# LeCAR-Lab/dial-mpc

Hardware: NVIDIA H100
Metric: sample-steps/s (Nsample*Hsample/wall-s) per MPC reverse_once, Go2 (higher is better)
Workload: dtype f32

## Files before the change

### dial_mpc_b200/csrc/dial_kernels.cu

```cuda
#include <cuda_runtime.h>
#include <stdio.h>
#include <stdlib.h>
#include <float.h>
#include <cmath>
#include <memory>
#include <string>
#include <vector>
#include <new>
#include "dial_host.h"
#define DIAL_STR2(x) #x
#define DIAL_STR(x) DIAL_STR2(x)

static thread_local std::string g_err;
static int fail(const std::string& s) { g_err = s; return -1; }
#define CUDA_OK(x) do { cudaError_t e_ = (x); if (e_ != cudaSuccess) return fail(std::string(#x) + ": " + cudaGetErrorString(e_)); } while (0)

#ifdef DIAL_ONLY_VARIANT
#define DIAL_HAS_VARIANT(v) ((v) == DIAL_ONLY_VARIANT)
#define DIAL_VARIANT DIAL_ONLY_VARIANT
#include "dial_rollout_variant.cu"
#else
#define DIAL_HAS_VARIANT(v) 1
#endif
#define DIAL_DECL_LAUNCH(v) cudaError_t dial_launch_rollout_v##v(const DevModel*, const DevPlan*, const RolloutArgs&, int, int, size_t, cudaStream_t);
// ... 346 lines not shown
  }
  if (tid == 0) {
    *counter = 0u;
    uint32_t n0, n1;
    split_rng(r0, r1, n0, n1);
    rng[0] = n0; rng[1] = n1;
    if (X.mbox) *X.seq = *X.seq + 1u;
  }
}

__global__ void mpc_split_kernel(uint32_t* __restrict__ rng, uint32_t* __restrict__ key) {
  if (threadIdx.x == 0) {
    const uint32_t k0 = rng[0], k1 = rng[1];
    uint32_t a0 = 0, b0 = 2, a1 = 1, b1 = 3;
    threefry2x32(k0, k1, a0, b0);
    threefry2x32(k0, k1, a1, b1);
    rng[0] = a0; rng[1] = a1; key[0] = b0; key[1] = b1;
  }
}

__global__ void mpc_shift_kernel(const float* __restrict__ Msh, const float* __restrict__ Yin,
                                 float* __restrict__ Yout, int n1, int nu) {
  const int i = threadIdx.x;
  Yin += (size_t)blockIdx.x * n1 * nu; Yout += (size_t)blockIdx.x * n1 * nu;
  if (i < n1 * nu) {
    const int k = i / nu, a = i - k * nu;
    float s = 0.f;
    for (int j = 0; j < n1; ++j) s += Msh[k * n1 + j] * Yin[j * nu + a];
    Yout[i] = s;
  }
}

#define TB_CHUNKS 32
struct TrajArgs {
  const float* traj[3];
  float* out[3];
  int ncol[3], coloff[3];
  int coltot, nrows, H;
  int inst_rows;
  const float* weights;
  int w_offset, mean_row, mean_weight_index, include_mean;
  float* partial;
};

template <bool BATCH>
__global__ void __launch_bounds__(256, 8) trajbar_partial_kernel(const TrajArgs T, const int32_t* __restrict__ iter_lim, int iter) {
  const int chunk = blockIdx.y, arr = BATCH ? blockIdx.z % 3 : blockIdx.z, inst = BATCH ? blockIdx.z / 3 : 0;
  const int ncol = arr == 0 ? T.ncol[0] : (arr == 1 ? T.ncol[1] : T.ncol[2]), len = T.H * ncol;
  const int coloff = arr == 0 ? T.coloff[0] : (arr == 1 ? T.coloff[1] : T.coloff[2]);
  const int j = blockIdx.x * 256 + threadIdx.x;
  if (blockIdx.x * 256 >= len || (BATCH && !schedule_runs(iter_lim, inst, iter))) return;
  const float* __restrict__ traj = (arr == 0 ? T.traj[0] : (arr == 1 ? T.traj[1] : T.traj[2])) + (size_t)inst * T.inst_rows * len;
  const float* wts = BATCH ? T.weights + (size_t)inst * (T.mean_weight_index + 1) : T.weights;
  const int per = (T.nrows + TB_CHUNKS - 1) / TB_CHUNKS;
  const int r0 = chunk * per, r1 = min(T.nrows, r0 + per);
  const int jj = j < len ? j : len - 1;
  float a = 0.f;
  for (int r = r0; r < r1; r += 8) {
    float wv[8], xv[8];
#pragma unroll
    for (int k = 0; k < 8; ++k) {
      const int rr = r + k;
      float wgt = 0.f;
      if (rr < r1) {
        if (rr == T.mean_row) wgt = T.include_mean ? wts[T.mean_weight_index] : 0.f;
        else wgt = wts[T.w_offset + rr];
      }
      wv[k] = wgt;
    }
#pragma unroll
    for (int k = 0; k < 8; ++k)
      xv[k] = (wv[k] != 0.f) ? traj[(size_t)(r + k) * len + jj] : 0.f;
#pragma unroll
    for (int k = 0; k < 8; ++k) a += wv[k] * xv[k];
  }
  if (j < len) {
    const int t = j / ncol, c = j - t * ncol;
    T.partial[(((size_t)inst * TB_CHUNKS + chunk) * T.H + t) * T.coltot + coloff + c] = a;
  }
}

template <bool BATCH>
__global__ void __launch_bounds__(128, 8) trajbar_final_kernel(const TrajArgs T, const int32_t* __restrict__ iter_lim, int iter) {
  const int t = blockIdx.x, inst = BATCH ? blockIdx.y : 0;
  if (BATCH && !schedule_runs(iter_lim, inst, iter)) return;
  const float* partial = T.partial + (size_t)inst * TB_CHUNKS * T.H * T.coltot;
  for (int col = threadIdx.x; col < T.coltot; col += blockDim.x) {
    float s = 0.f;
#pragma unroll 8
    for (int ch = 0; ch < TB_CHUNKS; ++ch) s += partial[((size_t)ch * T.H + t) * T.coltot + col];
    float* out; int ncol, off;
    if (col >= T.coloff[2]) { out = T.out[2]; ncol = T.ncol[2]; off = T.coloff[2]; }
    else if (col >= T.coloff[1]) { out = T.out[1]; ncol = T.ncol[1]; off = T.coloff[1]; }
    else { out = T.out[0]; ncol = T.ncol[0]; off = T.coloff[0]; }
    if (out) out[((size_t)inst * T.H + t) * ncol + (col - off)] = s;
  }
}

__global__ void __launch_bounds__(256) ensemble_reduce_kernel(const float* __restrict__ r, const EnsRisk* __restrict__ risk,
                                                              const EnsAdapt* __restrict__ adapt, const float* __restrict__ belief,
                                                              int K, int n1, float* __restrict__ rews,
                                                              const int32_t* __restrict__ iter_lim, int iter) {
  const int i = blockIdx.x * blockDim.x + threadIdx.x, b = blockIdx.y;
  if (i >= n1 || !schedule_runs(iter_lim, b, iter)) return;
  const EnsRisk R = risk[b];
  const float* rb = r + (size_t)b * K * n1 + i;
  rews[(size_t)b * n1 + i] = adapt[b].on ? ens_risk_reduce_weighted(rb, (size_t)n1, K, R, belief + (size_t)b * K, adapt[b].prune)
                                         : ens_risk_reduce(rb, (size_t)n1, K, R);
}

__global__ void __launch_bounds__(128) ens_gather_kernel(const float* __restrict__ Y, int K, int n1, int nu,
// ... 122 lines not shown
    ev.clear();
    cudaFree(d); cudaFreeHost(h);
    d = nullptr; h = nullptr;
  }
};

struct LaunchKey {
  bool models = false, members = false, sched = false, lims = false, adapt = false, delay = false, obs = false;
  bool predicts = false;
  int npred = 0;
  bool planning() const { return obs || npred > 0; }
  bool operator!=(const LaunchKey& o) const {
    return models != o.models || members != o.members || sched != o.sched || lims != o.lims || adapt != o.adapt ||
           delay != o.delay || obs != o.obs || predicts != o.predicts || npred != o.npred;
  }
};

struct dial_plan {
  DevModel hM;
  DevPlan hP;
  DevModel* dM = nullptr;
  DevPlan* dP = nullptr;
  int variant = 0;
  int shape = 0;
  int n_inst = 1;
  int n_ens = 0;
  int num_sms = 132;
  size_t smem_bytes = 0;
  float *traj_q[2] = {nullptr, nullptr}, *traj_qd[2] = {nullptr, nullptr}, *traj_x[2] = {nullptr, nullptr};
  int cur = 0;
  float* weights = nullptr;
  float* weights2 = nullptr;
  cudaStream_t side = nullptr;
  cudaEvent_t ev_main[2] = {nullptr, nullptr}, ev_side[2] = {nullptr, nullptr};
  float* partial = nullptr;
  float* tb_partial = nullptr;
  unsigned int* counter = nullptr;
  unsigned int* row_counter = nullptr;
  float* zeros = nullptr;
  int ybar_grid = 0;
  int upd_grid = 0;
  int64_t launches = 0;
  float* dbg = nullptr;
  dial_mpc_buffers mpc{};
  bool mpc_bound = false;
  float* mpc_Msh = nullptr;
  float* mpc_Y1 = nullptr;
  uint32_t* mpc_key = nullptr;
  struct MpcGraph { int n_diffuse, env_step, seen; cudaGraphExec_t exec; int64_t launches; };
  std::vector<MpcGraph> mpc_graphs;
  LaunchKey key, ran;
  Staged<DevModel> models;
  Staged<DevModel> members;
  float* ens_rews = nullptr;
  Staged<EnsRisk> risk;
  Staged<EnsAdapt> adapt;
  Staged<double> belief_L;
  Staged<float> belief_w;
  float* dEll = nullptr;
  float* pred_us = nullptr;
  float* pred_qd = nullptr;
  Staged<InstSchedule> sched;
  Staged<int32_t> lims;
  struct PlanningState {
    float *qpos = nullptr, *qvel = nullptr, *warm = nullptr;
    int32_t* cnt = nullptr;
// ... 57 lines not shown
static void fill_xch(const dial_plan* p, RolloutArgs& A) {
  if (!p->xch.on) return;
  A.xch_world = p->xch.world; A.xch_rank = p->xch.rank;
  for (int r = 0; r < p->xch.world; ++r) { A.xch_mbox[r] = p->xch.mbox(r); A.xch_flags[r] = p->xch.flags(r); }
  A.xch_seq = p->xch.seq(); A.xch_done = p->xch.done();
}
static XchWait xch_wait_args(const dial_plan* p, float* rews_copy) {
  XchWait X; memset(&X, 0, sizeof(X));
  if (p->xch.on) {
    X.mbox = p->xch.mbox(p->xch.rank); X.flags = p->xch.flags(p->xch.rank); X.seq = p->xch.seq(); X.err = p->xch.err();
    X.rews_copy = rews_copy; X.world = p->xch.world;
  }
  return X;
}

extern "C" int dial_abi_version(void) { return DIAL_ABI_VERSION; }
extern "C" const char* dial_last_error(void) { return g_err.c_str(); }
extern "C" size_t dial_sizeof(int which) {
  return which == 0 ? sizeof(dial_model_desc) : which == 1 ? sizeof(dial_plan_desc) : which == 2 ? sizeof(dial_state)
       : which == 3 ? sizeof(dial_mpc_buffers) : which == 4 ? sizeof(dial_task) : 0;
}

static cudaError_t launch_rollout(dial_plan* p, const RolloutArgs& A, int wpc, cudaStream_t st) {
  const size_t smem = sizeof(DevModel) + sizeof(DevPlan) + (size_t)wpc * p->hM.warp_floats * sizeof(float);
  int grid = (A.nrows + wpc - 1) / wpc;
  if (A.models && model_rows(A) > 0) grid = (A.nrows / model_rows(A)) * ((model_rows(A) + wpc - 1) / wpc);
  if (A.row_counter) {
    const int resident = p->num_sms * (wpc > 8 ? 1 : 16 / wpc);
    grid = grid < resident ? grid : resident;
    cudaError_t e = cudaMemsetAsync(A.row_counter, 0, sizeof(unsigned int), st);
    if (e != cudaSuccess) return e;
  }
  p->launches++;
#ifndef DIAL_ONLY_VARIANT
  if (p->shape > 0) return kShapes[p->shape - 1].launch(p->dM, p->dP, A, grid, wpc, smem, st);
#endif
  switch (p->variant) {
#if DIAL_HAS_VARIANT(1)
    case 1: return dial_launch_rollout_v1(p->dM, p->dP, A, grid, wpc, smem, st);
#endif
#if DIAL_HAS_VARIANT(2)
    case 2: return dial_launch_rollout_v2(p->dM, p->dP, A, grid, wpc, smem, st);
#endif
#if DIAL_HAS_VARIANT(3)
    case 3: return dial_launch_rollout_v3(p->dM, p->dP, A, grid, wpc, smem, st);
#endif
#if DIAL_HAS_VARIANT(4)
    case 4: return dial_launch_rollout_v4(p->dM, p->dP, A, grid, wpc, smem, st);
#endif
#if DIAL_HAS_VARIANT(0)
    case 0: return dial_launch_rollout_v0(p->dM, p->dP, A, grid, wpc, smem, st);
#endif
    default: return cudaErrorInvalidDeviceFunction;
  }
}

static int default_wpc(const dial_plan* p, int nrows) {
  const int per_sm = (nrows + p->num_sms - 1) / p->num_sms;
  const size_t fixed = sizeof(DevModel) + sizeof(DevPlan), slab = (size_t)p->hM.warp_floats * sizeof(float);
  int maxw = DIAL_MAXTHREADS / 32;
  while (maxw > 1 && fixed + maxw * slab > 227 * 1024) --maxw;
  if (per_sm <= maxw) return per_sm;
  const int waves = (per_sm + maxw - 1) / maxw;
  return (per_sm + waves - 1) / waves;
}

// ... 77 lines not shown
      if (kShapes[s].matches(p->hM, p->hP.c)) { p->shape = s + 1; break; }
#endif
  auto bad = [&](cudaError_t e, const char* what) {
    g_err = std::string(what) + ": " + cudaGetErrorString(e);
    dial_plan_destroy(p);
    return (dial_plan*)nullptr;
  };
  cudaError_t e = cudaSuccess;
  if (p->own(e, p->dM, sizeof(DevModel)) != cudaSuccess) return bad(e, "cudaMalloc(model)");
  if (p->own(e, p->dP, sizeof(DevPlan)) != cudaSuccess) return bad(e, "cudaMalloc(plan)");
  if ((e = cudaMemcpy(p->dM, &p->hM, sizeof(DevModel), cudaMemcpyHostToDevice)) != cudaSuccess) return bad(e, "cudaMemcpy(model)");
  if ((e = cudaMemcpy(p->dP, &p->hP, sizeof(DevPlan), cudaMemcpyHostToDevice)) != cudaSuccess) return bad(e, "cudaMemcpy(plan)");
  const size_t B = (size_t)p->n_inst, H = (size_t)c.Hsample + 1;
  const size_t rows = B * (p->n_ens > 1 ? (size_t)p->n_ens : 1) * ((size_t)c.Nsample + 1);
  const dial_model_desc& m = *model;
  for (int b = 0; b < 2; ++b) {
    if (p->own(e, p->traj_q[b], rows * H * m.nq * sizeof(float)) != cudaSuccess) return bad(e, "cudaMalloc(traj_q)");
    if (p->own(e, p->traj_qd[b], rows * H * m.nv * sizeof(float)) != cudaSuccess) return bad(e, "cudaMalloc(traj_qd)");
    if (p->own(e, p->traj_x[b], rows * H * 3 * (m.nbody - 1) * sizeof(float)) != cudaSuccess) return bad(e, "cudaMalloc(traj_x)");
  }
  if (p->n_ens > 1) {
    if (p->own(e, p->ens_rews, rows * sizeof(float)) != cudaSuccess) return bad(e, "cudaMalloc(ens_rews)");
    const size_t K = p->n_ens;
    const double L0 = log(1.0 / p->n_ens);
    if ((e = p->risk.allocate(B, 1, ens_risk_derive(p->n_ens, DIAL_ENS_MEAN, 1.f))) != cudaSuccess) return bad(e, "allocate(risk)");
    if ((e = p->adapt.allocate(B, 1, EnsAdapt{})) != cudaSuccess) return bad(e, "allocate(adapt)");
    if ((e = p->belief_L.allocate(B, K, L0)) != cudaSuccess) return bad(e, "allocate(belief)");
    if ((e = p->belief_w.allocate(B, K, (float)exp(L0))) != cudaSuccess) return bad(e, "allocate(belief)");
    if (p->own(e, p->dEll, B * K * sizeof(float)) != cudaSuccess) return bad(e, "cudaMalloc(belief)");
    if ((e = cudaMemset(p->dEll, 0, B * K * sizeof(float))) != cudaSuccess) return bad(e, "cudaMemset(belief)");
  }
  if (p->own(e, p->weights, B * ((size_t)c.Ntotal + 1) * sizeof(float)) != cudaSuccess) return bad(e, "cudaMalloc(weights)");
  if (p->own(e, p->weights2, B * ((size_t)c.Ntotal + 1) * sizeof(float)) != cudaSuccess) return bad(e, "cudaMalloc(weights2)");
  if ((e = cudaStreamCreateWithFlags(&p->side, cudaStreamNonBlocking)) != cudaSuccess) return bad(e, "cudaStreamCreate(side)");
  for (int i = 0; i < 2; ++i) {
    if ((e = cudaEventCreateWithFlags(&p->ev_main[i], cudaEventDisableTiming)) != cudaSuccess) return bad(e, "cudaEventCreate");
    if ((e = cudaEventCreateWithFlags(&p->ev_side[i], cudaEventDisableTiming)) != cudaSuccess) return bad(e, "cudaEventCreate");
  }
  const int ne = (c.Hnode + 1) * m.nu, slots = YBAR_THREADS / ne;
  int g = (c.Ntotal + 1 + slots - 1) / slots;
  p->ybar_grid = g < 1 ? 1 : (g > 2 * p->num_sms ? 2 * p->num_sms : g);
  {
    int gu = (c.Ntotal + 1 + slots * 8 - 1) / (slots * 8);
    p->upd_grid = gu < 1 ? 1 : (gu > p->ybar_grid ? p->ybar_grid : gu);
  }
  if (p->own(e, p->partial, B * p->ybar_grid * (ne + 1) * sizeof(float)) != cudaSuccess) return bad(e, "cudaMalloc(partial)");
  if (p->own(e, p->tb_partial, B * TB_CHUNKS * H * (m.nq + m.nv + 3 * (m.nbody - 1)) * sizeof(float)) != cudaSuccess) return bad(e, "cudaMalloc(tb_partial)");
  if (p->own(e, p->counter, B * sizeof(unsigned int)) != cudaSuccess) return bad(e, "cudaMalloc(counter)");
  if ((e = cudaMemset(p->counter, 0, B * sizeof(unsigned int))) != cudaSuccess) return bad(e, "cudaMemset(counter)");
  if (p->own(e, p->row_counter, sizeof(unsigned int)) != cudaSuccess) return bad(e, "cudaMalloc(row_counter)");
  if (getenv("DIAL_DEBUG_COUNTERS")) {
    if (p->own(e, p->dbg, 8 * sizeof(float)) != cudaSuccess) return bad(e, "cudaMalloc(dbg)");
    cudaMemset(p->dbg, 0, 8 * sizeof(float));
  }
  if (p->own(e, p->zeros, DIAL_MAXV * sizeof(float)) != cudaSuccess) return bad(e, "cudaMalloc(zeros)");
  if ((e = cudaMemset(p->zeros, 0, DIAL_MAXV * sizeof(float))) != cudaSuccess) return bad(e, "cudaMemset(zeros)");
  return p;
}

extern "C" void dial_plan_destroy(dial_plan* p) {
  if (!p) return;
  drop_graphs(p);
  for (int r = 0; r < DIAL_MAXRANK; ++r) {
    if (!p->xch.base[r]) continue;
    if (r == p->xch.rank) cudaFree(p->xch.base[r]); else cudaIpcCloseMemHandle(p->xch.base[r]);
  }
  cudaFree(p->xch.bars_partial);
// ... 511 lines not shown
  ybar_kernel<<<p->ybar_grid, YBAR_THREADS, 0, st>>>(w, eps, key ? key[0] : 0u, key ? key[1] : 0u, Ybar, noise_scale,
                                                     c.Ntotal, c.Hnode + 1, p->hM.m.nu, p->partial, p->counter, Ybar_out, nullptr);
  p->launches++;
  CUDA_OK(cudaGetLastError());
  if (weights && weights != p->weights)
    CUDA_OK(cudaMemcpyAsync(p->weights, weights, ((size_t)c.Ntotal + 1) * sizeof(float), cudaMemcpyDeviceToDevice, st));
  return 0;
}

static int launch_update(dial_plan* p, const float* rews, float* weights, const XchWait& X, uint32_t* rng,
                         const float* Ybar, const float* noise, float* Ybar_out, cudaStream_t st,
                         const InstSchedule* sched = nullptr, const int32_t* iter_lim = nullptr, int iter = 0,
                         const float* weights_prev = nullptr) {
  const dial_plan_desc& c = p->hP.c;
  update_kernel<<<dim3(p->upd_grid, p->n_inst), YBAR_THREADS, 0, st>>>(rews, c.Ntotal + 1, c.temp_sample, weights, X, rng, Ybar,
                                                                     noise, c.Ntotal, c.Hnode + 1, p->hM.m.nu, p->partial,
                                                                     p->counter, Ybar_out, sched, iter_lim, iter,
                                                                     weights_prev ? weights_prev : weights);
  p->launches++;
  CUDA_OK(cudaGetLastError());
  return 0;
}

extern "C" int dial_reverse_update_fused(dial_plan* p, const float* rews, uint32_t* rng, const float* Ybar,
                                         const float* noise_scale, float* Ybar_out, float* weights, void* stream) {
  if (!p || !rews || !rng || !Ybar || !noise_scale || !Ybar_out || !weights) return fail("dial_reverse_update_fused: null argument");
  const dial_plan_desc& c = p->hP.c;
  if (c.Ntotal != c.Nsample) return fail("dial_reverse_update_fused: sharded plans (Ntotal != Nsample) are not supported");
  if (c.Ntotal + 1 > (1 << 17)) return fail("dial_reverse_update_fused: needs Ntotal + 1 <= 131072 (the fused update)");
  XchWait X; memset(&X, 0, sizeof(X));
  return launch_update(p, rews, weights, X, rng, Ybar, noise_scale, Ybar_out, (cudaStream_t)stream);
}

static int enqueue_trajbar(dial_plan* p, const float* weights, int rank, float* qbar, float* qdbar, float* xbar,
                           cudaStream_t st, const int32_t* iter_lim = nullptr, int iter = 0) {
  const dial_plan_desc& c = p->hP.c;
  const dial_model_desc& m = p->hM.m;
  const float* w = weights ? weights : p->weights;
  const int H = c.Hsample + 1, rows = c.Nsample + 1;
  TrajArgs T;
  T.traj[0] = p->traj_q[p->cur]; T.traj[1] = p->traj_qd[p->cur]; T.traj[2] = p->traj_x[p->cur];
  T.out[0] = qbar; T.out[1] = qdbar; T.out[2] = xbar;
  const bool xsum = p->xch.on && qbar && qdbar && xbar;
  if (xsum) {
    T.out[0] = p->xch.bars_partial; T.out[1] = T.out[0] + (size_t)H * m.nq; T.out[2] = T.out[1] + (size_t)H * m.nv;
  }
  T.ncol[0] = m.nq; T.ncol[1] = m.nv; T.ncol[2] = 3 * (m.nbody - 1);
  T.coloff[0] = 0; T.coloff[1] = m.nq; T.coloff[2] = m.nq + m.nv;
  T.coltot = m.nq + m.nv + 3 * (m.nbody - 1);
  T.nrows = rows; T.inst_rows = (p->n_ens > 1 ? p->n_ens : 1) * rows; T.H = H; T.weights = w; T.w_offset = c.shard_offset; T.mean_row = c.Nsample;
  T.mean_weight_index = c.Ntotal; T.include_mean = rank == 0 ? 1 : 0; T.partial = p->tb_partial;
  const int maxlen = H * (T.ncol[2] > T.ncol[0] ? T.ncol[2] : T.ncol[0]);
  const dim3 g1((maxlen + 255) / 256, TB_CHUNKS, 3 * p->n_inst), g2(H, p->n_inst);
  const bool batch = p->n_inst > 1 || iter_lim;
  if (batch) trajbar_partial_kernel<true><<<g1, 256, 0, st>>>(T, iter_lim, iter);
  else trajbar_partial_kernel<false><<<g1, 256, 0, st>>>(T, nullptr, 0);
  p->launches++;
  CUDA_OK(cudaGetLastError());
  if (batch) trajbar_final_kernel<true><<<g2, 128, 0, st>>>(T, iter_lim, iter);
  else trajbar_final_kernel<false><<<g2, 128, 0, st>>>(T, nullptr, 0);
  p->launches++;
  CUDA_OK(cudaGetLastError());
  if (xsum) {
    BarsXch Bx; memset(&Bx, 0, sizeof(Bx));
    for (int r = 0; r < p->xch.world; ++r) { Bx.mbox[r] = p->xch.bars(r); Bx.flags[r] = p->xch.bflags(r); }
    Bx.seq = p->xch.bseq(); Bx.err = p->xch.err(); Bx.world = p->xch.world; Bx.rank = p->xch.rank; Bx.nbar = p->xch.nbar;
    Bx.partial = p->xch.bars_partial; Bx.out[0] = qbar; Bx.out[1] = qdbar; Bx.out[2] = xbar;
    Bx.n0 = H * m.nq; Bx.n1 = H * m.nv;
    bars_allreduce_kernel<<<1, 1024, 0, st>>>(Bx);
    p->launches++;
    CUDA_OK(cudaGetLastError());
  }
  return 0;
}

extern "C" int dial_reverse_trajbar(dial_plan* p, const float* weights, int rank, float* qbar, float* qdbar,
                                    float* xbar, void* stream) {
  if (!p) return fail("dial_reverse_trajbar: null plan");
  if (p->n_inst > 1) return fail("dial_reverse_trajbar: batched plans run through dial_mpc_step");
  return enqueue_trajbar(p, weights, rank, qbar, qdbar, xbar, (cudaStream_t)stream);
}

extern "C" int dial_exchange_create(dial_plan* p, int rank, int world, unsigned char handle_out[DIAL_IPC_HANDLE_BYTES]) {
  if (!p || !handle_out) return fail("dial_exchange_create: null argument");
  if (world < 2 || world > DIAL_MAXRANK || rank < 0 || rank >= world) return fail("dial_exchange_create: need 2 <= world <= DIAL_MAXRANK");
  static_assert(sizeof(cudaIpcMemHandle_t) <= DIAL_IPC_HANDLE_BYTES, "IPC handle does not fit");
  const dial_plan_desc& c = p->hP.c;
  const dial_model_desc& m = p->hM.m;
  if (c.Ntotal != c.Nsample * world || c.shard_offset != rank * c.Nsample) return fail("dial_exchange_create: plan shard does not match rank/world");
// ... 41 lines not shown
  if (!p || !out) return fail("dial_exchange_status: null argument");
  if (!p->xch.on) { for (int i = 0; i < 6; ++i) out[i] = 0; return 0; }
  CUDA_OK(cudaMemcpy(out, p->xch.base[p->xch.rank] + p->xch.o_local, 6 * sizeof(uint32_t), cudaMemcpyDeviceToHost));
  return 0;
}

extern "C" int dial_reverse_trajectories(dial_plan* p, float* q, float* qd, float* xpos, void* stream) {
  if (!p) return fail("dial_reverse_trajectories: null plan");
  if (p->n_inst > 1) return fail("dial_reverse_trajectories: batched plans run through dial_mpc_step");
  const dial_plan_desc& c = p->hP.c;
  const dial_model_desc& m = p->hM.m;
  const size_t n = ((size_t)c.Nsample + 1) * (c.Hsample + 1) * sizeof(float);
  cudaStream_t st = (cudaStream_t)stream;
  if (q) CUDA_OK(cudaMemcpyAsync(q, p->traj_q[p->cur], n * m.nq, cudaMemcpyDeviceToDevice, st));
  if (qd) CUDA_OK(cudaMemcpyAsync(qd, p->traj_qd[p->cur], n * m.nv, cudaMemcpyDeviceToDevice, st));
  if (xpos) CUDA_OK(cudaMemcpyAsync(xpos, p->traj_x[p->cur], n * 3 * (m.nbody - 1), cudaMemcpyDeviceToDevice, st));
  return 0;
}

extern "C" int dial_mpc_bind(dial_plan* p, const dial_mpc_buffers* b, const float* M_shift) {
  if (!p || !b || !M_shift) return fail("dial_mpc_bind: null argument");
  if (!b->qpos || !b->qvel || !b->qacc_warmstart || !b->counters || !b->rng || !b->Y || !b->ctrl || !b->reward ||
      !b->rews || !b->noise)
    return fail("dial_mpc_bind: only qbar/qdbar/xbar may be null");
  const dial_plan_desc& c = p->hP.c;
  if (c.Ntotal != c.Nsample && !p->xch.on)
    return fail("dial_mpc_bind: a sharded plan needs a connected exchange (dial_exchange_create / dial_exchange_connect) for the device-resident loop");
  if (c.Ntotal != c.Nsample && !b->rews_all) return fail("dial_mpc_bind: sharded plans need rews_all [Ntotal+1]");
  if (p->n_inst > 1 && b->rews_all) return fail("dial_mpc_bind: rews_all must be NULL on a batched plan");
  const int n1 = c.Hnode + 1, nu = p->hM.m.nu;
  drop_graphs(p);
  cudaError_t e = cudaSuccess;
  if (!p->mpc_Msh) CUDA_OK(p->own(e, p->mpc_Msh, DIAL_MAXNODE * DIAL_MAXNODE * sizeof(float)));
  if (!p->mpc_Y1) CUDA_OK(p->own(e, p->mpc_Y1, (size_t)p->n_inst * DIAL_MAXNODE * DIAL_MAXU * sizeof(float)));
  if (!p->mpc_key) CUDA_OK(p->own(e, p->mpc_key, 2 * sizeof(uint32_t)));
  CUDA_OK(cudaMemcpy(p->mpc_Msh, M_shift, (size_t)n1 * n1 * sizeof(float), cudaMemcpyHostToDevice));
  (void)nu;
  p->mpc = *b;
  p->mpc_bound = true;
  return 0;
}

static int mpc_enqueue(dial_plan* p, const LaunchKey& k, int n_diffuse, int env_step, cudaStream_t st) {
  const dial_plan_desc& c = p->hP.c;
  const dial_mpc_buffers& B = p->mpc;
  const int n1 = c.Hnode + 1, nu = p->hM.m.nu, ni = p->n_inst;
  const int K = p->n_ens > 1 ? p->n_ens : 1;
  const bool batched = ni > 1;
  const dial_plan::DelayQueue& Q = p->queue;
  const dial_plan::PlanningState& P = p->planning;
  float* Y[2] = {B.Y, p->mpc_Y1};
  int cur = 0;
  if (k.delay && (env_step == 1 || k.predicts)) {
    delay_queue_kernel<<<ni, 128, 0, st>>>(p->delay.d, Q.head, Q.ring, Y[cur], n1, nu, env_step == 1,
                                           Q.applied, Q.pending, Q.len);
    p->launches++;
    CUDA_OK(cudaGetLastError());
  }
  const float* act = k.delay ? Q.applied : Y[cur];
  const int act_n1 = k.delay ? 1 : n1;
  const bool adapt = env_step == 1 && k.adapt;
  if (adapt) {
    ens_gather_kernel<<<ni, 128, 0, st>>>(act, K, act_n1, nu, p->pred_us);
    p->launches++;
    CUDA_OK(cudaGetLastError());
    RolloutArgs A; memset(&A, 0, sizeof(A));
    A.qpos0 = B.qpos; A.qvel0 = B.qvel; A.warm0 = B.qacc_warmstart; A.counters_in = B.counters;
    A.nrows = ni * K; A.H = 1; A.mode = 0; A.us = p->pred_us;
    A.rows_per_inst = K; A.rows_per_model = 1; A.models = p->members.d;
    if (B.tasks) { A.tasks = B.tasks; A.task_rows = K; }
    A.qd = p->pred_qd;
    CUDA_OK(launch_rollout(p, A, 1, st));
  }
  if (env_step == 1) {
    RolloutArgs A; memset(&A, 0, sizeof(A));
    A.qpos0 = B.qpos; A.qvel0 = B.qvel; A.warm0 = B.qacc_warmstart;
    A.counters_in = B.counters; A.counters_out = B.counters;
    A.nrows = ni; A.H = 1; A.mode = 0; A.us = act; A.rewss = B.reward;
    if (batched) { A.rows_per_inst = 1; A.us_row = act_n1 * nu; }
    if (B.tasks) { A.tasks = B.tasks; A.task_rows = batched ? 1 : 0; }
    A.models = p->models.d;
    A.qpos_out = B.qpos; A.qvel_out = B.qvel; A.warm_out = B.qacc_warmstart; A.ctrl_out = B.ctrl;
    CUDA_OK(launch_rollout(p, A, 1, st));
  }
  if (adapt) {
    ens_belief_kernel<<<ni, 32, 0, st>>>(p->pred_qd, B.qvel, p->adapt.d, K, p->hM.m.nv, p->belief_L.d, p->belief_w.d, p->dEll);
    p->launches++;
    CUDA_OK(cudaGetLastError());
  }
  if (env_step == 1 || env_step == 2) {
    mpc_shift_kernel<<<ni, DIAL_MAXNODE * DIAL_MAXU, 0, st>>>(p->mpc_Msh, Y[cur], Y[cur ^ 1], n1, nu);
    p->launches++;
    CUDA_OK(cudaGetLastError());
    cur ^= 1;
  }
  const float *qpos0 = B.qpos, *qvel0 = B.qvel, *warm0 = B.qacc_warmstart;
  const int32_t* cnt0 = B.counters;
  if (k.obs) {
    observe_kernel<<<ni, 128, 0, st>>>(p->dM, p->obs.d, p->ob, p->delay.d, Q.pending, env_step == 1, B.qpos, B.qvel,
                                       B.qacc_warmstart, B.counters, act, act_n1 * nu, P.qpos, P.qvel, P.warm, P.cnt);
    p->launches++;
    CUDA_OK(cudaGetLastError());
  } else if (k.npred > 0) {
    const size_t nq = p->hM.m.nq, nv = p->hM.m.nv;
    CUDA_OK(cudaMemcpyAsync(P.qpos, B.qpos, ni * nq * sizeof(float), cudaMemcpyDeviceToDevice, st));
    CUDA_OK(cudaMemcpyAsync(P.qvel, B.qvel, ni * nv * sizeof(float), cudaMemcpyDeviceToDevice, st));
    CUDA_OK(cudaMemcpyAsync(P.warm, B.qacc_warmstart, ni * nv * sizeof(float), cudaMemcpyDeviceToDevice, st));
    CUDA_OK(cudaMemcpyAsync(P.cnt, B.counters, ni * 2 * sizeof(int32_t), cudaMemcpyDeviceToDevice, st));
  }
  for (int j = 0; j < k.npred; ++j) {
    RolloutArgs A; memset(&A, 0, sizeof(A));
    A.qpos0 = P.qpos; A.qvel0 = P.qvel; A.warm0 = P.warm;
    A.counters_in = P.cnt; A.counters_out = P.cnt;
    A.nrows = ni; A.H = 1; A.mode = 0; A.rows_per_inst = 1;
    A.us = (k.obs ? p->ob.seq : Q.pending) + (size_t)j * nu; A.us_row = DIAL_MAXDELAY * nu;
    if (B.tasks) { A.tasks = B.tasks; A.task_rows = batched ? 1 : 0; }
    A.models = p->n_ens > 0 ? P.models : p->models.d;
    A.iter_lim = k.obs ? p->ob.len : Q.len; A.iter = j;
    A.qpos_out = P.qpos; A.qvel_out = P.qvel; A.warm_out = P.warm;
    CUDA_OK(launch_rollout(p, A, 1, st));
  }
  if (k.planning()) { qpos0 = P.qpos; qvel0 = P.qvel; warm0 = P.warm; cnt0 = P.cnt; }
  const bool bars = B.qbar && B.qdbar && B.xbar;
  float* wts[2] = {p->weights, p->weights2};
  const size_t nw = (size_t)ni * (c.Ntotal + 1);
  for (int i = 0; i < n_diffuse; ++i) {
    const float* noise = B.noise + (size_t)i * n1;
    const bool fused = c.Ntotal + 1 <= (1 << 17) && !getenv("DIAL_NO_FUSED_UPDATE");
    if (!fused) {
      mpc_split_kernel<<<1, 32, 0, st>>>(B.rng, p->mpc_key);
      p->launches++;
      CUDA_OK(cudaGetLastError());
    }
    if (bars && i >= 2) CUDA_OK(cudaStreamWaitEvent(st, p->ev_side[i & 1], 0));
    RolloutArgs A; memset(&A, 0, sizeof(A));
    A.qpos0 = qpos0; A.qvel0 = qvel0; A.warm0 = warm0; A.counters_in = cnt0;
    A.nrows = ni * K * (c.Nsample + 1); A.H = c.Hsample + 1; A.mode = 1;
    if (batched || p->n_ens > 0) A.rows_per_inst = K * (c.Nsample + 1);
    if (B.tasks) { A.tasks = B.tasks; A.task_rows = batched ? K * (c.Nsample + 1) : 0; }
    if (p->n_ens > 0) { A.rows_per_model = c.Nsample + 1; A.models = p->members.d; }
    else A.models = p->models.d;
    A.Ybar = Y[cur]; A.noise = noise;
    A.sched = p->sched.d; A.iter_lim = p->lims.d; A.iter = i;
    if (fused) A.rng_dev = B.rng; else A.key_dev = p->mpc_key;
    p->cur ^= 1;
    A.rews = K > 1 ? p->ens_rews : B.rews; A.q = p->traj_q[p->cur]; A.qd = p->traj_qd[p->cur]; A.xpos = p->traj_x[p->cur];
    A.dbg = p->dbg;
    fill_xch(p, A);
    CUDA_OK(launch_rollout_any(p, A, st));
    if (K > 1) {
      const dim3 grid((c.Nsample + 1 + 255) / 256, ni);
      ensemble_reduce_kernel<<<grid, 256, 0, st>>>(p->ens_rews, p->risk.d, p->adapt.d, p->belief_w.d, K, c.Nsample + 1, B.rews,
                                                   p->lims.d, i);
      p->launches++;
      CUDA_OK(cudaGetLastError());
    }
    float* w = wts[i & 1];
    XchWait X = xch_wait_args(p, B.rews_all);
    if (fused) {
      int rc = launch_update(p, B.rews, w, X, B.rng, Y[cur], noise, Y[cur ^ 1], st, p->sched.d, p->lims.d, i,
                             wts[i > 0 ? (i - 1) & 1 : 0]);
      if (rc) return rc;
    } else {
      weights_kernel<<<1, 1024, 0, st>>>(B.rews, c.Ntotal + 1, c.temp_sample, w, X);
      p->launches++;
      CUDA_OK(cudaGetLastError());
      ybar_kernel<<<p->ybar_grid, YBAR_THREADS, 0, st>>>(w, nullptr, 0u, 0u, Y[cur], noise, c.Ntotal, n1, nu,
                                                         p->partial, p->counter, Y[cur ^ 1], p->mpc_key);
      p->launches++;
      CUDA_OK(cudaGetLastError());
    }
    cur ^= 1;
    if (bars) {
      CUDA_OK(cudaEventRecord(p->ev_main[i & 1], st));
      CUDA_OK(cudaStreamWaitEvent(p->side, p->ev_main[i & 1], 0));
      int rc = enqueue_trajbar(p, w, p->xch.on ? p->xch.rank : 0, B.qbar, B.qdbar, B.xbar, p->side, p->lims.d, i);
      if (rc) return rc;
      CUDA_OK(cudaEventRecord(p->ev_side[i & 1], p->side));
    }
  }
  if (cur != 0) CUDA_OK(cudaMemcpyAsync(Y[0], Y[1], (size_t)ni * n1 * nu * sizeof(float), cudaMemcpyDeviceToDevice, st));
  if (bars && n_diffuse > 0) {
    if (n_diffuse >= 2) CUDA_OK(cudaStreamWaitEvent(st, p->ev_side[(n_diffuse - 2) & 1], 0));
    CUDA_OK(cudaStreamWaitEvent(st, p->ev_side[(n_diffuse - 1) & 1], 0));
  }
  if (n_diffuse > 0 && wts[(n_diffuse - 1) & 1] != p->weights)
    CUDA_OK(cudaMemcpyAsync(p->weights, p->weights2, nw * sizeof(float), cudaMemcpyDeviceToDevice, st));
  return 0;
}

extern "C" int dial_mpc_step(dial_plan* p, int n_diffuse, int env_step, void* stream) {
  if (!p) return fail("dial_mpc_step: null plan");
  if (!p->mpc_bound) return fail("dial_mpc_step: call dial_mpc_bind first");
  if (n_diffuse < 0 || n_diffuse > 64) return fail("dial_mpc_step: n_diffuse out of range");
  if (env_step < 0 || env_step > 2) return fail("dial_mpc_step: env_step must be 0 (plan only), 1 (env step + shift) or 2 (shift only)");
  if (p->n_inst > 1 && getenv("DIAL_NO_FUSED_UPDATE")) return fail("dial_mpc_step: batched plans need the fused update (unset DIAL_NO_FUSED_UPDATE)");
  if ((p->sched.d || p->lims.d) && getenv("DIAL_NO_FUSED_UPDATE"))
    return fail("dial_mpc_step: per-instance schedules and iteration limits need the fused update (unset DIAL_NO_FUSED_UPDATE)");
  for (int b = 0; p->sched.d && b < p->n_inst; ++b) {
    const InstSchedule& S = p->sched.h[b];
    const int runs = p->lims.d && p->lims.h[b] < n_diffuse ? p->lims.h[b] : n_diffuse;
    if (S.on && runs > S.n_rows)
      return fail("dial_mpc_step: instance " + std::to_string(b) + " runs " + std::to_string(runs) +
                  " diffusion iterations, its schedule has " + std::to_string(S.n_rows) + " rows");
  }
  cudaStream_t st = (cudaStream_t)stream;
  if (p->key != p->ran) drop_graphs(p);
  p->ran = p->key;
  dial_plan::MpcGraph* g = nullptr;
  for (auto& e : p->mpc_graphs) if (e.n_diffuse == n_diffuse && e.env_step == env_step) g = &e;
  if (!g) {
    p->mpc_graphs.push_back({n_diffuse, env_step, 1, nullptr, 0});
    return mpc_enqueue(p, p->ran, n_diffuse, env_step, st);
  }
  if (!g->exec) {
    if (getenv("DIAL_NO_GRAPH")) return mpc_enqueue(p, p->ran, n_diffuse, env_step, st);
    cudaStream_t cs;
    CUDA_OK(cudaStreamCreateWithFlags(&cs, cudaStreamNonBlocking));
    const int64_t l0 = p->launches;
    cudaError_t e = cudaStreamBeginCapture(cs, cudaStreamCaptureModeThreadLocal);
    if (e != cudaSuccess) { cudaStreamDestroy(cs); CUDA_OK(e); }
    int rc = mpc_enqueue(p, p->ran, n_diffuse, env_step, cs);
    cudaGraph_t graph = nullptr;
    e = cudaStreamEndCapture(cs, &graph);
    cudaStreamDestroy(cs);
    g->launches = p->launches - l0;
    p->launches = l0;
    if (rc) { if (graph) cudaGraphDestroy(graph); return rc; }
    CUDA_OK(e);
    e = cudaGraphInstantiate(&g->exec, graph, 0);
    cudaGraphDestroy(graph);
    CUDA_OK(e);
  }
  CUDA_OK(cudaGraphLaunch(g->exec, st));
  p->launches += g->launches;
  return 0;
}

extern "C" void dial_key_split(const uint32_t key[2], uint32_t out0[2], uint32_t out1[2]) {
  uint32_t a0 = 0, b0 = 2, a1 = 1, b1 = 3;
  threefry2x32(key[0], key[1], a0, b0);
  threefry2x32(key[0], key[1], a1, b1);
  out0[0] = a0; out0[1] = a1; out1[0] = b0; out1[1] = b1;
}

extern "C" int dial_solver_variant(const dial_model_desc* model) {
  if (!model) return fail("null descriptor");
  DevModel* D = new (std::nothrow) DevModel();
  if (!D) return fail("out of memory");
  std::string err;
  int v = -1;
  if (!derive_model(*model, *D, err)) g_err = err;
  else if ((v = star_variant(*D)) < 0) g_err = "this build instantiates the dense (elliptic) solver path for nv = " DIAL_STR(DIAL_DENSE_NV) " only (custom builds: dial_mpc_b200.custom compiles it for the model's nv)";
  delete D;
  return v;
}

extern "C" const char* dial_plan_rollout_kernel(const dial_plan* p) {
  static const char* const generic[] = {"v0", "v1", "v2", "v3", "v4"};
  if (!p) return "";
#ifndef DIAL_ONLY_VARIANT
  if (p->shape > 0) return kShapes[p->shape - 1].name;
#endif
// ... 70 lines not shown
```

Measured before the change: 76.20 million.

## Overlap trajectory-bar reduction with rollout via stream priorities and persistent CTAs

Turns the trajbar partial kernel into a grid-stride persistent kernel that stages weights in shared memory, and sizes its grid to fill only the SMs the rollout leaves idle. The side stream gets low priority and the main graph stream high priority (with node-priority graph instantiation), so the bar reductions stay off the rollout's critical path. Y buffers are ping-ponged with parity planning so the final result lands in B.Y, and the weights tail copy is removed by picking buffers by parity. This adds more complex buffer indexing and depends on the scheduler honouring priorities.

```diff
diff --git a/dial_mpc_b200/csrc/dial_kernels.cu b/dial_mpc_b200/csrc/dial_kernels.cu
--- a/dial_mpc_b200/csrc/dial_kernels.cu
+++ b/dial_mpc_b200/csrc/dial_kernels.cu
@@ -402,6 +402,7 @@
 }
 
 #define TB_CHUNKS 32
+#define TB_TILE 256
 struct TrajArgs {
   const float* traj[3];
   float* out[3];
@@ -411,42 +412,55 @@
   const float* weights;
   int w_offset, mean_row, mean_weight_index, include_mean;
   float* partial;
+  int nblk, items;
 };
 
 template <bool BATCH>
-__global__ void __launch_bounds__(256, 8) trajbar_partial_kernel(const TrajArgs T, const int32_t* __restrict__ iter_lim, int iter) {
-  const int chunk = blockIdx.y, arr = BATCH ? blockIdx.z % 3 : blockIdx.z, inst = BATCH ? blockIdx.z / 3 : 0;
-  const int ncol = arr == 0 ? T.ncol[0] : (arr == 1 ? T.ncol[1] : T.ncol[2]), len = T.H * ncol;
-  const int coloff = arr == 0 ? T.coloff[0] : (arr == 1 ? T.coloff[1] : T.coloff[2]);
-  const int j = blockIdx.x * 256 + threadIdx.x;
-  if (blockIdx.x * 256 >= len || (BATCH && !schedule_runs(iter_lim, inst, iter))) return;
-  const float* __restrict__ traj = (arr == 0 ? T.traj[0] : (arr == 1 ? T.traj[1] : T.traj[2])) + (size_t)inst * T.inst_rows * len;
-  const float* wts = BATCH ? T.weights + (size_t)inst * (T.mean_weight_index + 1) : T.weights;
-  const int per = (T.nrows + TB_CHUNKS - 1) / TB_CHUNKS;
-  const int r0 = chunk * per, r1 = min(T.nrows, r0 + per);
-  const int jj = j < len ? j : len - 1;
-  float a = 0.f;
-  for (int r = r0; r < r1; r += 8) {
-    float wv[8], xv[8];
+__global__ void __launch_bounds__(TB_TILE, 4) trajbar_partial_kernel(const TrajArgs T, const int32_t* __restrict__ iter_lim, int iter) {
+  __shared__ float ws[TB_TILE];
+  for (int item = blockIdx.x; item < T.items; item += gridDim.x) {
+    const int bx = item % T.nblk, rest = item / T.nblk, chunk = rest % TB_CHUNKS, z = rest / TB_CHUNKS;
+    const int arr = BATCH ? z % 3 : z, inst = BATCH ? z / 3 : 0;
+    const int ncol = arr == 0 ? T.ncol[0] : (arr == 1 ? T.ncol[1] : T.ncol[2]), len = T.H * ncol;
+    const int coloff = arr == 0 ? T.coloff[0] : (arr == 1 ? T.coloff[1] : T.coloff[2]);
+    const int j = bx * TB_TILE + threadIdx.x;
+    if (bx * TB_TILE >= len || (BATCH && !schedule_runs(iter_lim, inst, iter))) continue;
+    const float* __restrict__ traj = (arr == 0 ? T.traj[0] : (arr == 1 ? T.traj[1] : T.traj[2])) + (size_t)inst * T.inst_rows * len;
+    const float* wts = BATCH ? T.weights + (size_t)inst * (T.mean_weight_index + 1) : T.weights;
+    const int per = (T.nrows + TB_CHUNKS - 1) / TB_CHUNKS;
+    const int r0 = chunk * per, r1 = min(T.nrows, r0 + per);
+    const int jj = j < len ? j : len - 1;
+    float a = 0.f;
+    for (int t0 = r0; t0 < r1; t0 += TB_TILE) {
+      const int nt = min(TB_TILE, r1 - t0);
+      __syncthreads();
+      {
+        const int rr = t0 + threadIdx.x;
+        float wgt = 0.f;
+        if (threadIdx.x < nt) {
+          if (rr == T.mean_row) wgt = T.include_mean ? wts[T.mean_weight_index] : 0.f;
+          else wgt = wts[T.w_offset + rr];
+        }
+        ws[threadIdx.x] = wgt;
+      }
+      __syncthreads();
+      for (int g = 0; g < nt; g += 16) {
+        float xv[16];
 #pragma unroll
-    for (int k = 0; k < 8; ++k) {
-      const int rr = r + k;
-      float wgt = 0.f;
-      if (rr < r1) {
-        if (rr == T.mean_row) wgt = T.include_mean ? wts[T.mean_weight_index] : 0.f;
-        else wgt = wts[T.w_offset + rr];
+        for (int k = 0; k < 16; ++k)
+          xv[k] = (ws[g + k] != 0.f) ? traj[(size_t)(t0 + g + k) * len + jj] : 0.f;
+#pragma unroll
+        for (int k = 0; k < 8; ++k) a += ws[g + k] * xv[k];
+        if (g + 8 < nt) {
+#pragma unroll
+          for (int k = 8; k < 16; ++k) a += ws[g + k] * xv[k];
+        }
       }
-      wv[k] = wgt;
     }
-#pragma unroll
-    for (int k = 0; k < 8; ++k)
-      xv[k] = (wv[k] != 0.f) ? traj[(size_t)(r + k) * len + jj] : 0.f;
-#pragma unroll
-    for (int k = 0; k < 8; ++k) a += wv[k] * xv[k];
-  }
-  if (j < len) {
-    const int t = j / ncol, c = j - t * ncol;
-    T.partial[(((size_t)inst * TB_CHUNKS + chunk) * T.H + t) * T.coltot + coloff + c] = a;
+    if (j < len) {
+      const int t = j / ncol, c = j - t * ncol;
+      T.partial[(((size_t)inst * TB_CHUNKS + chunk) * T.H + t) * T.coltot + coloff + c] = a;
+    }
   }
 }
 
@@ -635,6 +649,9 @@
   float* weights = nullptr;
   float* weights2 = nullptr;
   cudaStream_t side = nullptr;
+  int prio_main = 0;
+  bool bars_legacy = false;
+  int roll_grid = 0, roll_wpc = 0;
   cudaEvent_t ev_main[2] = {nullptr, nullptr}, ev_side[2] = {nullptr, nullptr};
   float* partial = nullptr;
   float* tb_partial = nullptr;
@@ -758,6 +775,7 @@
     if (e != cudaSuccess) return e;
   }
   p->launches++;
+  p->roll_grid = grid; p->roll_wpc = wpc;
 #ifndef DIAL_ONLY_VARIANT
   if (p->shape > 0) return kShapes[p->shape - 1].launch(p->dM, p->dP, A, grid, wpc, smem, st);
 #endif
@@ -901,7 +919,13 @@
   }
   if (p->own(e, p->weights, B * ((size_t)c.Ntotal + 1) * sizeof(float)) != cudaSuccess) return bad(e, "cudaMalloc(weights)");
   if (p->own(e, p->weights2, B * ((size_t)c.Ntotal + 1) * sizeof(float)) != cudaSuccess) return bad(e, "cudaMalloc(weights2)");
-  if ((e = cudaStreamCreateWithFlags(&p->side, cudaStreamNonBlocking)) != cudaSuccess) return bad(e, "cudaStreamCreate(side)");
+  {
+    int least = 0, greatest = 0;
+    if ((e = cudaDeviceGetStreamPriorityRange(&least, &greatest)) != cudaSuccess) return bad(e, "cudaDeviceGetStreamPriorityRange");
+    p->bars_legacy = getenv("DIAL_BARS_LEGACY") != nullptr;
+    p->prio_main = p->bars_legacy ? least : greatest;
+    if ((e = cudaStreamCreateWithPriority(&p->side, cudaStreamNonBlocking, least)) != cudaSuccess) return bad(e, "cudaStreamCreate(side)");
+  }
   for (int i = 0; i < 2; ++i) {
     if ((e = cudaEventCreateWithFlags(&p->ev_main[i], cudaEventDisableTiming)) != cudaSuccess) return bad(e, "cudaEventCreate");
     if ((e = cudaEventCreateWithFlags(&p->ev_side[i], cudaEventDisableTiming)) != cudaSuccess) return bad(e, "cudaEventCreate");
@@ -1479,8 +1503,14 @@
   return launch_update(p, rews, weights, X, rng, Ybar, noise_scale, Ybar_out, (cudaStream_t)stream);
 }
 
+static int bars_ctas_beside_rollout(const dial_plan* p) {
+  const long regs = (long)p->roll_wpc * 32 * (65536 / DIAL_MAXTHREADS) + 65536 / 4;
+  if (p->bars_legacy || p->roll_grid >= p->num_sms || regs <= 65536) return 0;
+  return p->num_sms - p->roll_grid;
+}
+
 static int enqueue_trajbar(dial_plan* p, const float* weights, int rank, float* qbar, float* qdbar, float* xbar,
-                           cudaStream_t st, const int32_t* iter_lim = nullptr, int iter = 0) {
+                           cudaStream_t st, const int32_t* iter_lim = nullptr, int iter = 0, int ctas = 0) {
   const dial_plan_desc& c = p->hP.c;
   const dial_model_desc& m = p->hM.m;
   const float* w = weights ? weights : p->weights;
@@ -1498,10 +1528,13 @@
   T.nrows = rows; T.inst_rows = (p->n_ens > 1 ? p->n_ens : 1) * rows; T.H = H; T.weights = w; T.w_offset = c.shard_offset; T.mean_row = c.Nsample;
   T.mean_weight_index = c.Ntotal; T.include_mean = rank == 0 ? 1 : 0; T.partial = p->tb_partial;
   const int maxlen = H * (T.ncol[2] > T.ncol[0] ? T.ncol[2] : T.ncol[0]);
-  const dim3 g1((maxlen + 255) / 256, TB_CHUNKS, 3 * p->n_inst), g2(H, p->n_inst);
+  T.nblk = (maxlen + TB_TILE - 1) / TB_TILE;
+  T.items = T.nblk * TB_CHUNKS * 3 * p->n_inst;
+  const int g1 = ctas > 0 && ctas < T.items ? ctas : T.items;
+  const dim3 g2(H, p->n_inst);
   const bool batch = p->n_inst > 1 || iter_lim;
-  if (batch) trajbar_partial_kernel<true><<<g1, 256, 0, st>>>(T, iter_lim, iter);
-  else trajbar_partial_kernel<false><<<g1, 256, 0, st>>>(T, nullptr, 0);
+  if (batch) trajbar_partial_kernel<true><<<g1, TB_TILE, 0, st>>>(T, iter_lim, iter);
+  else trajbar_partial_kernel<false><<<g1, TB_TILE, 0, st>>>(T, nullptr, 0);
   p->launches++;
   CUDA_OK(cudaGetLastError());
   if (batch) trajbar_final_kernel<true><<<g2, 128, 0, st>>>(T, iter_lim, iter);
@@ -1609,7 +1642,7 @@
   drop_graphs(p);
   cudaError_t e = cudaSuccess;
   if (!p->mpc_Msh) CUDA_OK(p->own(e, p->mpc_Msh, DIAL_MAXNODE * DIAL_MAXNODE * sizeof(float)));
-  if (!p->mpc_Y1) CUDA_OK(p->own(e, p->mpc_Y1, (size_t)p->n_inst * DIAL_MAXNODE * DIAL_MAXU * sizeof(float)));
+  if (!p->mpc_Y1) CUDA_OK(p->own(e, p->mpc_Y1, 2 * (size_t)p->n_inst * DIAL_MAXNODE * DIAL_MAXU * sizeof(float)));
   if (!p->mpc_key) CUDA_OK(p->own(e, p->mpc_key, 2 * sizeof(uint32_t)));
   CUDA_OK(cudaMemcpy(p->mpc_Msh, M_shift, (size_t)n1 * n1 * sizeof(float), cudaMemcpyHostToDevice));
   (void)nu;
@@ -1626,15 +1659,22 @@
   const bool batched = ni > 1;
   const dial_plan::DelayQueue& Q = p->queue;
   const dial_plan::PlanningState& P = p->planning;
-  float* Y[2] = {B.Y, p->mpc_Y1};
-  int cur = 0;
+  const int hops = (env_step == 1 || env_step == 2 ? 1 : 0) + n_diffuse;
+  int hop = 0;
+  float* y = B.Y;
+  auto next_y = [&]() -> float* {
+    ++hop;
+    if (hops == 1) return p->mpc_Y1;
+    if (hop == 1 && (hops & 1)) return p->mpc_Y1 + (size_t)ni * DIAL_MAXNODE * DIAL_MAXU;
+    return ((hops - hop) & 1) ? p->mpc_Y1 : B.Y;
+  };
   if (k.delay && (env_step == 1 || k.predicts)) {
-    delay_queue_kernel<<<ni, 128, 0, st>>>(p->delay.d, Q.head, Q.ring, Y[cur], n1, nu, env_step == 1,
+    delay_queue_kernel<<<ni, 128, 0, st>>>(p->delay.d, Q.head, Q.ring, y, n1, nu, env_step == 1,
                                            Q.applied, Q.pending, Q.len);
     p->launches++;
     CUDA_OK(cudaGetLastError());
   }
-  const float* act = k.delay ? Q.applied : Y[cur];
+  const float* act = k.delay ? Q.applied : y;
   const int act_n1 = k.delay ? 1 : n1;
   const bool adapt = env_step == 1 && k.adapt;
   if (adapt) {
@@ -1666,10 +1706,11 @@
     CUDA_OK(cudaGetLastError());
   }
   if (env_step == 1 || env_step == 2) {
-    mpc_shift_kernel<<<ni, DIAL_MAXNODE * DIAL_MAXU, 0, st>>>(p->mpc_Msh, Y[cur], Y[cur ^ 1], n1, nu);
+    float* y_out = next_y();
+    mpc_shift_kernel<<<ni, DIAL_MAXNODE * DIAL_MAXU, 0, st>>>(p->mpc_Msh, y, y_out, n1, nu);
     p->launches++;
     CUDA_OK(cudaGetLastError());
-    cur ^= 1;
+    y = y_out;
   }
   const float *qpos0 = B.qpos, *qvel0 = B.qvel, *warm0 = B.qacc_warmstart;
   const int32_t* cnt0 = B.counters;
@@ -1699,8 +1740,7 @@
   }
   if (k.planning()) { qpos0 = P.qpos; qvel0 = P.qvel; warm0 = P.warm; cnt0 = P.cnt; }
   const bool bars = B.qbar && B.qdbar && B.xbar;
-  float* wts[2] = {p->weights, p->weights2};
-  const size_t nw = (size_t)ni * (c.Ntotal + 1);
+  auto wts = [&](int i) { return ((n_diffuse - 1 - i) & 1) ? p->weights2 : p->weights; };
   for (int i = 0; i < n_diffuse; ++i) {
     const float* noise = B.noise + (size_t)i * n1;
     const bool fused = c.Ntotal + 1 <= (1 << 17) && !getenv("DIAL_NO_FUSED_UPDATE");
@@ -1717,7 +1757,7 @@
     if (B.tasks) { A.tasks = B.tasks; A.task_rows = batched ? K * (c.Nsample + 1) : 0; }
     if (p->n_ens > 0) { A.rows_per_model = c.Nsample + 1; A.models = p->members.d; }
     else A.models = p->models.d;
-    A.Ybar = Y[cur]; A.noise = noise;
+    A.Ybar = y; A.noise = noise;
     A.sched = p->sched.d; A.iter_lim = p->lims.d; A.iter = i;
     if (fused) A.rng_dev = B.rng; else A.key_dev = p->mpc_key;
     p->cur ^= 1;
@@ -1732,37 +1772,37 @@
       p->launches++;
       CUDA_OK(cudaGetLastError());
     }
-    float* w = wts[i & 1];
+    float* w = wts(i);
+    float* y_out = next_y();
     XchWait X = xch_wait_args(p, B.rews_all);
     if (fused) {
-      int rc = launch_update(p, B.rews, w, X, B.rng, Y[cur], noise, Y[cur ^ 1], st, p->sched.d, p->lims.d, i,
-                             wts[i > 0 ? (i - 1) & 1 : 0]);
+      int rc = launch_update(p, B.rews, w, X, B.rng, y, noise, y_out, st, p->sched.d, p->lims.d, i,
+                             i > 0 ? wts(i - 1) : p->weights);
       if (rc) return rc;
     } else {
       weights_kernel<<<1, 1024, 0, st>>>(B.rews, c.Ntotal + 1, c.temp_sample, w, X);
       p->launches++;
       CUDA_OK(cudaGetLastError());
-      ybar_kernel<<<p->ybar_grid, YBAR_THREADS, 0, st>>>(w, nullptr, 0u, 0u, Y[cur], noise, c.Ntotal, n1, nu,
-                                                         p->partial, p->counter, Y[cur ^ 1], p->mpc_key);
+      ybar_kernel<<<p->ybar_grid, YBAR_THREADS, 0, st>>>(w, nullptr, 0u, 0u, y, noise, c.Ntotal, n1, nu,
+                                                         p->partial, p->counter, y_out, p->mpc_key);
       p->launches++;
       CUDA_OK(cudaGetLastError());
     }
-    cur ^= 1;
+    y = y_out;
     if (bars) {
       CUDA_OK(cudaEventRecord(p->ev_main[i & 1], st));
       CUDA_OK(cudaStreamWaitEvent(p->side, p->ev_main[i & 1], 0));
-      int rc = enqueue_trajbar(p, w, p->xch.on ? p->xch.rank : 0, B.qbar, B.qdbar, B.xbar, p->side, p->lims.d, i);
+      const int ctas = i + 1 < n_diffuse ? bars_ctas_beside_rollout(p) : 0;
+      int rc = enqueue_trajbar(p, w, p->xch.on ? p->xch.rank : 0, B.qbar, B.qdbar, B.xbar, p->side, p->lims.d, i, ctas);
       if (rc) return rc;
       CUDA_OK(cudaEventRecord(p->ev_side[i & 1], p->side));
     }
   }
-  if (cur != 0) CUDA_OK(cudaMemcpyAsync(Y[0], Y[1], (size_t)ni * n1 * nu * sizeof(float), cudaMemcpyDeviceToDevice, st));
+  if (y != B.Y) CUDA_OK(cudaMemcpyAsync(B.Y, y, (size_t)ni * n1 * nu * sizeof(float), cudaMemcpyDeviceToDevice, st));
   if (bars && n_diffuse > 0) {
     if (n_diffuse >= 2) CUDA_OK(cudaStreamWaitEvent(st, p->ev_side[(n_diffuse - 2) & 1], 0));
     CUDA_OK(cudaStreamWaitEvent(st, p->ev_side[(n_diffuse - 1) & 1], 0));
   }
-  if (n_diffuse > 0 && wts[(n_diffuse - 1) & 1] != p->weights)
-    CUDA_OK(cudaMemcpyAsync(p->weights, p->weights2, nw * sizeof(float), cudaMemcpyDeviceToDevice, st));
   return 0;
 }
 
@@ -1793,7 +1833,7 @@
   if (!g->exec) {
     if (getenv("DIAL_NO_GRAPH")) return mpc_enqueue(p, p->ran, n_diffuse, env_step, st);
     cudaStream_t cs;
-    CUDA_OK(cudaStreamCreateWithFlags(&cs, cudaStreamNonBlocking));
+    CUDA_OK(cudaStreamCreateWithPriority(&cs, cudaStreamNonBlocking, p->prio_main));
     const int64_t l0 = p->launches;
     cudaError_t e = cudaStreamBeginCapture(cs, cudaStreamCaptureModeThreadLocal);
     if (e != cudaSuccess) { cudaStreamDestroy(cs); CUDA_OK(e); }
@@ -1805,7 +1845,7 @@
     p->launches = l0;
     if (rc) { if (graph) cudaGraphDestroy(graph); return rc; }
     CUDA_OK(e);
-    e = cudaGraphInstantiate(&g->exec, graph, 0);
+    e = cudaGraphInstantiate(&g->exec, graph, p->bars_legacy ? 0 : cudaGraphInstantiateFlagUseNodePriority);
     cudaGraphDestroy(graph);
     CUDA_OK(e);
   }
```

Result: faster. 77.11 million, median of 6 (+1.2%).
